# flock-lab/flock

Hardware: AMD Instinct MI355X
Metric: NEXMark rows/sec per node (q3 join, q5 agg) (higher is better)
Workload: dtype int32; 1 GPU; NEXMark q5 hopping(10,5) over 1087 s x 1000000 events/s per GPU; query=q5, input_rows_per_gpu=1000040000, windows_per_gpu=216, parallelism=one GPU, one process

## Files before the change

flock_amd/csrc/q5.hip:

```cpp
#include <algorithm>

#include "sort.hpp"

using namespace flockgpu;

namespace {

constexpr int kQ5Iters = 8;
constexpr int kQ5Tile = kBlock * 4 * kQ5Iters;
constexpr int kHist = 4096;
constexpr int kHistPad = 64;
constexpr int kSlots = kHist / 2;
constexpr int kSlotBits = 11;
static_assert(kSlots == (1 << kSlotBits), "slot bits");
constexpr int kLdsMaxProbe = 24;
constexpr uint32_t kFib = 0x9E3779B1u;
constexpr int kHotMin = 16;
constexpr int kMaxWinPanes = 8;
constexpr uint32_t kWideTile = 0x40000000u;

using u16x2 = unsigned short __attribute__((ext_vector_type(2)));
__device__ __forceinline__ u16x2 as_u16x2(uint32_t w) { return __builtin_bit_cast(u16x2, w); }
__device__ __forceinline__ u16x2 nonzero_u16x2(u16x2 c) {
    uint32_t r;
// ... 835 lines not shown
            const u16x2 one = {1, 1};
            u16x2 pk_a = {0, 0}, pk_b = {0, 0};
            uint32_t sum32 = 0;
            const uint32_t i_first = blockIdx.x * kBlock + threadIdx.x, i_step = gridDim.x * kBlock;
            for (uint32_t i = i_first; i < ng; i += i_step) {
                const int64_t k0 = pd.base + (int64_t)i * G;
                const uint64_t idx = (uint64_t)(k0 - next.base);
                const bool cov = act_b && idx < (uint64_t)next.range;
                const uint4 m4 = *reinterpret_cast<const uint4 *>(mine + (uint64_t)i * 4);
                uint4 o4 = *reinterpret_cast<const uint4 *>(theirs + (cov ? idx / 2 : uint64_t(0)));
                o4.x = cov ? o4.x : 0u;
                o4.y = cov ? o4.y : 0u;
                o4.z = cov ? o4.z : 0u;
                o4.w = cov ? o4.w : 0u;
                const uint32_t mw[4] = {m4.x, m4.y, m4.z, m4.w}, ow[4] = {o4.x, o4.y, o4.z, o4.w};
#pragma unroll
                for (int j = 0; j < 4; ++j) sum32 = __builtin_amdgcn_udot2(as_u16x2(mw[j]), one, sum32, false);
                if (act_b) {
#pragma unroll
                    for (int j = 0; j < 4; ++j) {
                        const u16x2 c = __builtin_elementwise_add_sat(as_u16x2(mw[j]), as_u16x2(ow[j]));
                        pk_b = __builtin_elementwise_max(pk_b, c);
                        groups_b = __builtin_amdgcn_udot2(nonzero_u16x2(c), one, groups_b, false);
                    }
                }
                if (act_a && !((uint64_t)(k0 - prev.base) < (uint64_t)prev.range)) {
#pragma unroll
                    for (int j = 0; j < 4; ++j) {
                        const u16x2 c = as_u16x2(mw[j]);
                        pk_a = __builtin_elementwise_max(pk_a, c);
                        groups_a = __builtin_amdgcn_udot2(nonzero_u16x2(c), one, groups_a, false);
                    }
                }
            }
            sum = sum32;
            best_a = max((uint32_t)pk_a.x, (uint32_t)pk_a.y);
            best_b = max((uint32_t)pk_b.x, (uint32_t)pk_b.y);
            if (best_b == 0xFFFFu) {
                for (uint32_t i = i_first; i < ng; i += i_step) {
                    const uint64_t idx = (uint64_t)(pd.base + (int64_t)i * G - next.base);
                    if (!(idx < (uint64_t)next.range)) continue;
                    uint32_t me[G], o[G];
                    unpack(*reinterpret_cast<const uint4 *>(mine + (uint64_t)i * 4), me);
                    unpack(*reinterpret_cast<const uint4 *>(theirs + idx / 2), o);
#pragma unroll
                    for (int j = 0; j < G; ++j) best_b = max(best_b, me[j] + o[j]);
                }
            }
        }
    }
    if (!packed_done)
    for (uint32_t i = blockIdx.x * kBlock + threadIdx.x; i < ng; i += gridDim.x * kBlock) {
        const int64_t k0 = pd.base + (int64_t)i * G;
        uint32_t me[G];
        unpack(*reinterpret_cast<const uint4 *>(mine + (uint64_t)i * 4), me);
        if (k16 && !SELECT) {
#pragma unroll
            for (int j = 0; j < G; ++j) sum += me[j];
        }
        if (act_b) {
            uint32_t c[G];
#pragma unroll
            for (int j = 0; j < G; ++j) c[j] = me[j];
            const uint64_t idx = (uint64_t)(k0 - next.base);
            if (idx < (uint64_t)next.range) {
                uint32_t o[G];
                unpack(*reinterpret_cast<const uint4 *>(theirs + (k16 ? idx / 2 : idx)), o);
#pragma unroll
                for (int j = 0; j < G; ++j) c[j] += o[j];
            }
            if (tab_b) {
#pragma unroll
                for (int j = 0; j < G; ++j) c[j] += table_find(tb, cap, (uint32_t)(int32_t)(k0 + j));
            }
#pragma unroll
            for (int j = 0; j < G; ++j) take(c[j], (int32_t)(k0 + j), wb, mx_b, best_b, groups_b);
        }
        if (act_a && !((uint64_t)(k0 - prev.base) < (uint64_t)prev.range)) {
            uint32_t c[G];
#pragma unroll
            for (int j = 0; j < G; ++j) c[j] = me[j];
            if (tab_a) {
#pragma unroll
                for (int j = 0; j < G; ++j) c[j] += table_find(ta, cap, (uint32_t)(int32_t)(k0 + j));
            }
#pragma unroll
            for (int j = 0; j < G; ++j) take(c[j], (int32_t)(k0 + j), wa, mx_a, best_a, groups_a);
        }
    }
    if (tab_b && act_b) {
        for (uint32_t sl = blockIdx.x * kBlock + threadIdx.x; sl < cap; sl += gridDim.x * kBlock) {
            const uint64_t e = tb[sl];
            if (!e) continue;
            const int64_t key = (int32_t)(uint32_t)(e >> 32);
            if ((uint64_t)(key - pd.base) < (uint64_t)pd.range || (uint64_t)(key - next.base) < (uint64_t)next.range) continue;
            if (SELECT) {
                if ((uint32_t)e == mx_b) {
                    const uint32_t pos = atomicAdd(cursor, 1u);
                    if (pos < out_cap) {
                        out_win[pos] = wb;
                        out_key[pos] = (int32_t)key;
                    }
                }
            } else {
                best_b = max(best_b, (uint32_t)e);
                groups_b += 1;
            }
        }
    }
    if (!SELECT) {
        const uint32_t ba = wave_max_u32(best_a), bb = wave_max_u32(best_b);
        const uint64_t ga = wave_sum_u64(groups_a), gb = wave_sum_u64(groups_b), gs = k16 ? wave_sum_u64(sum) : 0;
        if (lane_id() == 0) {
            s_best[0][threadIdx.x >> 6] = ba;
            s_best[1][threadIdx.x >> 6] = bb;
            s_groups[0][threadIdx.x >> 6] = ga;
            s_groups[1][threadIdx.x >> 6] = gb;
            s_groups[2][threadIdx.x >> 6] = gs;
        }
        __syncthreads();
        if (threadIdx.x < 2) {
            const int r = threadIdx.x;
            const int32_t w = r == 0 ? wa : wb;
            uint32_t b = 0;
            uint64_t g = 0;
#pragma unroll
            for (int v = 0; v < kWavesPerBlock; ++v) {
                b = max(b, s_best[r][v]);
                g += s_groups[r][v];
            }
            if (w >= 0) {
                if (b) block_max[((size_t)w * 2 + (r == 0 ? 1 : 0)) * gridDim.x + blockIdx.x] = b;
                if (b) atomicMax(reinterpret_cast<unsigned long long *>(&win_max[w]), (unsigned long long)b);
                if (g) atomicAdd(reinterpret_cast<unsigned long long *>(&win_groups[w]), (unsigned long long)g);
            }
        }
        if (k16 && threadIdx.x == 2) {
            uint64_t t = 0;
#pragma unroll
            for (int v = 0; v < kWavesPerBlock; ++v) t += s_groups[2][v];
            if (t) atomicAdd(&pane_sum[p], (unsigned long long)t);
        }
    }
}

constexpr int kFinishThreads = 1024;
constexpr uint32_t kFinishMax = 1024;
__global__ __launch_bounds__(kFinishThreads) void q5_finish_kernel(const uint64_t *__restrict__ meta, uint32_t n_meta, int32_t n_win, const uint64_t *__restrict__ info,
                                                                   const int32_t *__restrict__ slow_list, const int32_t *__restrict__ sel_win,
                                                                   const int32_t *__restrict__ sel_key, uint32_t out_cap, int32_t *__restrict__ out_auction,
                                                                   uint64_t *__restrict__ out_num, uint64_t *__restrict__ h_fin,
                                                                   const unsigned long long *__restrict__ pane_sum, const unsigned long long *__restrict__ tab_rows,
                                                                   const int64_t *__restrict__ seg_off, const int32_t *__restrict__ pane_win_ptr, int32_t n_panes) {
    __shared__ uint64_t s_k[kFinishMax];
    __shared__ uint32_t s_bad;
    const uint32_t *tail = reinterpret_cast<const uint32_t *>(meta + 2 * (size_t)n_win);
    const uint32_t n_sel = tail[0], err = tail[1];
    if (threadIdx.x == 0) s_bad = 0;
    __syncthreads();
    if (pane_sum && (!info || info[2]))
        for (int32_t p = threadIdx.x; p < n_panes; p += kFinishThreads)
            if (pane_win_ptr[p + 1] != pane_win_ptr[p] && pane_sum[p] + tab_rows[p] != (unsigned long long)(seg_off[2 * p + 1] - seg_off[2 * p])) s_bad = 1;
    __syncthreads();
    const uint32_t bad16 = s_bad;
    for (uint32_t i = threadIdx.x; i < n_meta; i += kFinishThreads) h_fin[i] = meta[i];
    if (threadIdx.x < 3) h_fin[n_meta + threadIdx.x] = info ? info[threadIdx.x] : 0;
    if (threadIdx.x == 3) h_fin[n_meta + 3] = (uint64_t)(uint32_t)slow_list[0] | ((uint64_t)bad16 << 32);
    const bool sortable = !err && !bad16 && n_sel <= kFinishMax && n_sel <= out_cap && (!info || info[2]);
    if (threadIdx.x == 4) h_fin[n_meta + 4] = sortable ? 1 : 0;
    int64_t *h_off = reinterpret_cast<int64_t *>(h_fin + n_meta + 5);
    if (!sortable) return;
    uint32_t p2 = 1;
    while (p2 < n_sel) p2 <<= 1;
    if (threadIdx.x < p2)
        s_k[threadIdx.x] = threadIdx.x < n_sel ? ((uint64_t)(uint32_t)sel_win[threadIdx.x] << 32) | ((uint32_t)sel_key[threadIdx.x] ^ 0x80000000u) : ~0ull;
    __syncthreads();
    for (uint32_t k = 2; k <= p2; k <<= 1)
        for (uint32_t j = k >> 1; j > 0; j >>= 1) {
            const uint32_t i = threadIdx.x, l = i ^ j;
            if (i < p2 && l > i) {
                const uint64_t a = s_k[i], b = s_k[l];
                const bool up = (i & k) == 0;
                if ((a > b) == up) {
                    s_k[i] = b;
                    s_k[l] = a;
                }
            }
            __syncthreads();
        }
    if (threadIdx.x < n_sel) {
        const uint64_t e = s_k[threadIdx.x];
        out_auction[threadIdx.x] = (int32_t)((uint32_t)e ^ 0x80000000u);
        out_num[threadIdx.x] = meta[(uint32_t)(e >> 32)];
    }
    for (int32_t w = threadIdx.x; w <= n_win; w += kFinishThreads) {
        uint32_t lo = 0, hi = n_sel;
        while (lo < hi) {
            const uint32_t mid = (lo + hi) >> 1;
            if ((int32_t)(s_k[mid] >> 32) < w) lo = mid + 1;
            else hi = mid;
        }
        h_off[w] = (int64_t)lo;
    }
}

constexpr int kPartItems = 16;
constexpr int kPartTile = kBlock * kPartItems;
constexpr int kPartShift = 13;
constexpr int kPartMaxDigits = 256;

__device__ __forceinline__ uint32_t part_digit(int32_t key, const PaneDesc &pd, uint32_t straggler) {
    const uint64_t idx = (uint64_t)((int64_t)key - pd.base);
    return idx < (uint64_t)pd.range ? (uint32_t)(idx >> kPartShift) : straggler;
}

__global__ __launch_bounds__(kBlock) void q5_part_tile_kernel(const int32_t *__restrict__ auction, SegTiles st, const PaneDesc *__restrict__ panes,
                                                              const int32_t *__restrict__ pane_win_ptr, uint32_t nd, int32_t *__restrict__ off_mat,
                                                              int32_t *__restrict__ keys_out, uint16_t *__restrict__ low_out,
                                                              uint32_t *__restrict__ sample) {
    __shared__ uint32_t s_cnt[kPartMaxDigits];
    __shared__ __attribute__((aligned(16))) uint16_t s_low[kPartTile];
    __shared__ uint32_t s_wave_total[kWavesPerBlock];
    __shared__ int32_t s_red[2 * kWavesPerBlock];
    const int lane = lane_id(), wave = threadIdx.x >> 6;
    s_cnt[threadIdx.x] = 0;
    const int32_t tile = (int32_t)blockIdx.x;
    const TileRange tr = locate_tile(st, tile, kPartTile);
    if (pane_win_ptr[tr.seg] == pane_win_ptr[tr.seg + 1]) return;
    const int32_t t0 = st.tile_first[tr.seg], tiles_p = st.tile_first[tr.seg + 1] - t0;
    int32_t *off = off_mat + (size_t)t0 * (nd + 1) + (tile - t0);
    const PaneDesc pd = panes[tr.seg];
    int32_t k[kPartItems];
#pragma unroll
    for (int it = 0; it < kPartItems / 4; ++it) {
        const int64_t r0 = tr.tile_begin + (int64_t)(it * kBlock + threadIdx.x) * 4;
        if (r0 >= tr.lo && r0 + 4 <= tr.hi) {
            const int4 t = stream_load4(auction + r0);
            k[it * 4 + 0] = t.x; k[it * 4 + 1] = t.y; k[it * 4 + 2] = t.z; k[it * 4 + 3] = t.w;
        } else {
#pragma unroll
            for (int j = 0; j < 4; ++j) k[it * 4 + j] = (r0 + j >= tr.lo && r0 + j < tr.hi) ? auction[r0 + j] : 0;
        }
    }
    __syncthreads();
    uint16_t rank[kPartItems];
    int32_t mn = 0x7fffffff, mx = (int32_t)0x80000000;
#pragma unroll
    for (int i = 0; i < kPartItems; ++i) {
        const int64_t r = tr.tile_begin + (int64_t)((i >> 2) * kBlock + threadIdx.x) * 4 + (i & 3);
        rank[i] = 0;
        if (r >= tr.lo && r < tr.hi) {
            rank[i] = (uint16_t)atomicAdd(&s_cnt[part_digit(k[i], pd, nd - 1)], 1u);
            mn = min(mn, k[i]);
            mx = max(mx, k[i]);
        }
    }
    __syncthreads();
    {
        const uint32_t c = s_cnt[threadIdx.x];
        const uint32_t in = wave_incl_scan_u32(c);
        if (lane == 63) s_wave_total[wave] = in;
        __syncthreads();
        uint32_t o = in - c;
#pragma unroll
        for (int w = 0; w < kWavesPerBlock; ++w) o += w < wave ? s_wave_total[w] : 0u;
        s_cnt[threadIdx.x] = o;
        if (threadIdx.x < nd) off[(size_t)threadIdx.x * tiles_p] = (int32_t)o;
        if (threadIdx.x == 0) off[(size_t)nd * tiles_p] = (int32_t)(tr.hi - tr.lo);
    }
    __syncthreads();
#pragma unroll
    for (int i = 0; i < kPartItems; ++i) {
        const int64_t r = tr.tile_begin + (int64_t)((i >> 2) * kBlock + threadIdx.x) * 4 + (i & 3);
        if (r >= tr.lo && r < tr.hi) {
            const uint32_t d = part_digit(k[i], pd, nd - 1), pos = s_cnt[d] + rank[i];
            if (d == nd - 1) keys_out[(size_t)tile * kPartTile + pos] = k[i];
            else s_low[pos] = (uint16_t)(((uint32_t)k[i] - (uint32_t)pd.base) & ((1u << kPartShift) - 1));
        }
    }
    __syncthreads();
    {
        const uint4 *src = reinterpret_cast<const uint4 *>(s_low);
        uint4 *dst = reinterpret_cast<uint4 *>(low_out + (size_t)tile * kPartTile);
        const uint32_t n16 = ((uint32_t)(tr.hi - tr.lo) + 7u) >> 3;
        for (uint32_t i = threadIdx.x; i < n16; i += kBlock) stream_store4(dst + i, src[i]);
    }
    if ((blockIdx.x & 63u) == 0) {
#pragma unroll
        for (int o = 32; o > 0; o >>= 1) {
            mn = min(mn, __shfl_xor(mn, o, 64));
            mx = max(mx, __shfl_xor(mx, o, 64));
        }
        if (lane == 0) {
            s_red[wave] = mn;
            s_red[kWavesPerBlock + wave] = mx;
        }
        __syncthreads();
        if (threadIdx.x == 0) {
            for (int w = 1; w < kWavesPerBlock; ++w) {
                mn = min(mn, s_red[w]);
                mx = max(mx, s_red[kWavesPerBlock + w]);
            }
            atomicAdd(&sample[0], 1u);
            if (mx >= mn && (uint32_t)mx - (uint32_t)mn < (uint32_t)kHist / 2) atomicAdd(&sample[1], 1u);
        }
    }
}

__global__ __launch_bounds__(kBlock) void q5_bucket_count_kernel(const int32_t *__restrict__ keys, const uint16_t *__restrict__ low, SegTiles st,
                                                                 const PaneDesc *__restrict__ panes,
                                                                 const int32_t *__restrict__ pane_win_ptr, const int32_t *__restrict__ pane_win_idx,
                                                                 uint32_t nd, const int32_t *__restrict__ off_mat, uint32_t *counters, uint64_t *tables,
                                                                 uint32_t cap, uint32_t *tab_used, uint32_t *err) {
    __shared__ uint32_t s_hist[1 << kPartShift];
    const uint32_t d = blockIdx.x;
    const int32_t p = blockIdx.y;
    const int32_t t0 = st.tile_first[p], tiles_p = st.tile_first[p + 1] - t0;
    if (tiles_p == 0 || pane_win_ptr[p] == pane_win_ptr[p + 1]) return;
    const int32_t *lo_row = off_mat + (size_t)t0 * (nd + 1) + (size_t)d * tiles_p, *hi_row = lo_row + tiles_p;
    const PaneDesc pd = panes[p];
    const int lane = lane_id(), wave = threadIdx.x >> 6;
    if (d == nd - 1) {
        FlushArgs f;
        f.wp0 = pane_win_ptr[p];
        f.wp1 = pane_win_ptr[p + 1];
        f.pane = pd;
        f.pane_win_idx = pane_win_idx;
        f.counters = counters;
        f.tables = tables;
        f.cap = cap;
        f.tab_used = tab_used;
        f.err = err;
        for (int32_t t = wave; t < tiles_p; t += kWavesPerBlock) {
            const int32_t a = lo_row[t], b = hi_row[t];
            for (int32_t i = a + lane; i < b; i += 64) emit_pair(keys[(size_t)(t0 + t) * kPartTile + i], 1u, f);
        }
        return;
    }
    {
        uint4 *z = reinterpret_cast<uint4 *>(s_hist);
        for (int i = threadIdx.x; i < (1 << kPartShift) / 4; i += kBlock) z[i] = make_uint4(0, 0, 0, 0);
    }
    __syncthreads();
    auto add = [&](uint32_t bin, bool valid) {
        const uint32_t hot = __builtin_amdgcn_readfirstlane(bin);
        const uint64_t b = __ballot(valid && bin == hot);
        if (valid && bin == hot) {
            if (mbcnt(b) == 0) atomicAdd(&s_hist[hot], (uint32_t)__popcll((unsigned long long)b));
        } else if (valid) {
            atomicAdd(&s_hist[bin], 1u);
        }
    };
// ... 180 lines not shown
        now.insert(now.end(), idx.begin(), idx.end());
        if (sig != now) {
            std::copy(ptr.begin(), ptr.end(), h_ptr);
            std::copy(idx.begin(), idx.end(), h_idx);
            std::copy(role_a.begin(), role_a.end(), h_roles);
            std::copy(role_b.begin(), role_b.end(), h_roles + role_a.size());
            FG_HIP(ctx, hipMemcpyAsync(d_ptr, h_ptr, ptr.size() * sizeof(int32_t), hipMemcpyHostToDevice, ctx->stream));
            if (!idx.empty())
                FG_HIP(ctx, hipMemcpyAsync(d_idx, h_idx, idx.size() * sizeof(int32_t), hipMemcpyHostToDevice, ctx->stream));
            FG_HIP(ctx, hipMemcpyAsync(d_roles, h_roles, 2 * role_a.size() * sizeof(int32_t), hipMemcpyHostToDevice, ctx->stream));
            sig = now;
        }
    }

    int32_t *d_rng = nullptr, *h_rng = nullptr;
    const size_t n_rng = (size_t)2 * kRangeBlocks * std::max(n_panes, 1);
    FG_TRY(arena_get_t(ctx, "q5.pane_range", n_rng + 2, &d_rng));
    FG_TRY(pinned_get_t(ctx, "q5.pane_range", n_rng + 2, &h_rng));
    std::vector<PaneDesc> panes((size_t)std::max(n_panes, 1));
    std::vector<WinDesc> wins((size_t)std::max(n_win, 1));
    for (auto &p : panes) p = PaneDesc{0, 0, 0, 0};
    for (int w = 0; w < n_win; ++w) wins[w] = WinDesc{0, 0, win->win_pane_lo[w], win->win_pane_hi[w], 0};
    uint64_t cnt_total = 0, scan_total = 0;
    bool dense = st.n_tiles > 0 && n_win > 0 && max_win_panes <= kMaxWinPanes;
    std::vector<int64_t> &hint = ctx->host_i64[weight ? "q5.layout_hint.weighted" : "q5.layout_hint"];
    if (hint.size() != 3) hint.assign(3, 0);
    const uint64_t budget = std::max<uint64_t>(uint64_t(256) << 20, (uint64_t)covered_rows * 4 * 2);
    if (dense) {
        LaunchScope ls(ctx, "q5_range_kernel");
        hipLaunchKernelGGL(q5_range_kernel, dim3(kRangeBlocks, (unsigned)n_panes), dim3(kBlock), 0, ctx->stream, auction, rows, st.seg_off, d_rng);
    }
    FG_TRY(check_launch(ctx, "q5_range_kernel"));
    std::vector<int64_t> &wide_hint = ctx->host_i64["q5.wide_hint"];
    if (wide_hint.size() != 1) wide_hint.assign(1, 0);
    bool wide_mode = wide_hint[0] != 0 && !weight && !part && dense;
    bool wide_ran = false;
    bool speculate = dense && !part && hint[2] && hint[0] > 0 && !wide_mode;
    auto host_layout = [&]() -> int {
        FG_HIP(ctx, hipMemcpyAsync(h_rng, d_rng, sizeof(int32_t) * n_rng, hipMemcpyDeviceToHost, ctx->stream));
        FG_HIP(ctx, hipStreamSynchronize(ctx->stream));
        cnt_total = scan_total = 0;
        for (int p = 0; p < n_panes && dense; ++p) {
            if (ptr[p + 1] == ptr[p] || se[p] <= sb[p]) continue;
            int64_t lo = INT64_MAX, hi = INT64_MIN;
            for (int b = 0; b < kRangeBlocks; ++b) {
                lo = std::min<int64_t>(lo, h_rng[((size_t)p * kRangeBlocks + b) * 2]);
                hi = std::max<int64_t>(hi, h_rng[((size_t)p * kRangeBlocks + b) * 2 + 1]);
            }
            if (lo > hi) continue;
            int64_t base = 0, range = 0;
            if (!q5_pane_layout(lo, hi, &base, &range)) { dense = false; break; }
            panes[p] = PaneDesc{base, cnt_total, (uint32_t)range, 0};
            cnt_total += (uint64_t)range;
        }
        for (int w = 0; w < n_win && dense; ++w) {
            int64_t lo = INT64_MAX, hi = INT64_MIN;
            for (int p = win->win_pane_lo[w]; p < win->win_pane_hi[w]; ++p)
                if (panes[p].range) {
                    lo = std::min(lo, panes[p].base);
                    hi = std::max(hi, panes[p].base + (int64_t)panes[p].range);
                }
            if (lo >= hi) continue;
            if (hi - lo >= (int64_t(1) << 31)) { dense = false; break; }
            wins[w].base = lo;
            wins[w].range = (uint32_t)(hi - lo);
            scan_total += (uint64_t)(hi - lo);
        }
        if (dense && (cnt_total * 4 > budget || scan_total * 4 > 2 * budget)) dense = false;
        return FLOCKGPU_OK;
    };
    if (dense && !speculate) FG_TRY(host_layout());
    PaneDesc *d_panes = nullptr, *h_panes = nullptr;
    WinDesc *d_wins = nullptr, *h_wins = nullptr;
    FG_TRY(arena_get_t(ctx, "q5.panes", panes.size(), &d_panes));
    FG_TRY(pinned_get_t(ctx, "q5.panes", panes.size(), &h_panes));
    FG_TRY(arena_get_t(ctx, "q5.wins", wins.size(), &d_wins));
    FG_TRY(pinned_get_t(ctx, "q5.wins", wins.size(), &h_wins));
    uint64_t *d_info = nullptr, *h_info = nullptr;
    FG_TRY(arena_get_t(ctx, "q5.layout_info", 4, &d_info));
    FG_TRY(pinned_get_t(ctx, "q5.layout_info", 4, &h_info));
    auto upload_layout = [&]() -> int {
        if (!dense) {
            cnt_total = scan_total = 0;
            for (auto &p : panes) p = PaneDesc{0, 0, 0, 0};
            for (int w = 0; w < n_win; ++w) wins[w] = WinDesc{0, 0, win->win_pane_lo[w], win->win_pane_hi[w], 0};
        }
        std::copy(panes.begin(), panes.end(), h_panes);
        std::copy(wins.begin(), wins.end(), h_wins);
        ctx->host_i64["q5.wins_sig"].clear();
        FG_HIP(ctx, hipMemcpyAsync(d_panes, h_panes, panes.size() * sizeof(PaneDesc), hipMemcpyHostToDevice, ctx->stream));
        FG_HIP(ctx, hipMemcpyAsync(d_wins, h_wins, wins.size() * sizeof(WinDesc), hipMemcpyHostToDevice, ctx->stream));
        return FLOCKGPU_OK;
    };
    uint32_t *counters = nullptr;
    uint64_t capacity = 0;
    std::vector<int64_t> &preclean = ctx->host_i64["q5.preclean"];
    if (preclean.size() != 2) preclean.assign(2, 0);
    LayoutArgs lay{};
    uint64_t clean_upto = 0;
    const bool c16 = !weight && !part && !wide_mode && hop2 && ctx->host_i64["q5.no_c16"].empty();
    auto words_of = [&](uint64_t n_counters) -> uint64_t { return c16 ? (n_counters + 1) / 2 : n_counters; };
    if (speculate) {
        FG_TRY(arena_get_t(ctx, "q5.counters", (size_t)words_of((uint64_t)hint[0] + (uint64_t)hint[0] / 8) + 8, &counters));
        capacity = (ctx->arena["q5.counters"].cap / sizeof(uint32_t) - 8) * (c16 ? 2 : 1);
        if (preclean[0] == (int64_t)reinterpret_cast<uintptr_t>(counters)) clean_upto = (uint64_t)preclean[1];
        {
            std::vector<int64_t> &wsig = ctx->host_i64["q5.wins_sig"];
            std::vector<int64_t> wnow;
            wnow.reserve((size_t)2 * n_win + 2);
            wnow.push_back((int64_t)reinterpret_cast<uintptr_t>(d_wins));
            for (int w = 0; w < n_win; ++w) {
                wnow.push_back(win->win_pane_lo[w]);
                wnow.push_back(win->win_pane_hi[w]);
            }
            if (wsig != wnow) {
                std::copy(wins.begin(), wins.end(), h_wins);
                FG_HIP(ctx, hipMemcpyAsync(d_wins, h_wins, wins.size() * sizeof(WinDesc), hipMemcpyHostToDevice, ctx->stream));
                wsig = wnow;
            }
        }
        lay = LayoutArgs{d_rng, d_ptr, st.seg_off, n_panes, n_win, capacity, budget, d_panes, d_wins, d_info};
        cnt_total = (uint64_t)hint[0];
        scan_total = (uint64_t)hint[1];
    } else {
        FG_TRY(upload_layout());
        FG_TRY(arena_get_t(ctx, "q5.counters", (size_t)words_of(cnt_total) + 8, &counters));
    }
    preclean[0] = preclean[1] = 0;

    const size_t n_meta = (size_t)2 * n_win + 1 + ((size_t)n_win + 1) / 2 + 1;
    const size_t n_meta_all = n_meta + (size_t)2 * std::max(n_panes, 0);
    uint64_t *d_meta = nullptr, *h_meta = nullptr;
    FG_TRY(arena_get_t(ctx, "q5.meta", n_meta_all, &d_meta));
    unsigned long long *d_pane_sum = reinterpret_cast<unsigned long long *>(d_meta + n_meta), *d_tab_rows = d_pane_sum + std::max(n_panes, 0);
    FG_TRY(pinned_get_t(ctx, "q5.meta", n_meta, &h_meta));
    uint32_t *d_cursor = reinterpret_cast<uint32_t *>(d_meta + 2 * n_win), *d_err = d_cursor + 1, *d_used = d_cursor + 2;

    unsigned long long *d_wsum = nullptr, *h_wsum = nullptr;
    if (weight && n_panes > 0) {
        FG_TRY(arena_get_t(ctx, "q5.pane_weight", (size_t)n_panes + 1, &d_wsum));
        FG_TRY(pinned_get_t(ctx, "q5.pane_weight", (size_t)n_panes + 1, &h_wsum));
    }
    double rpg = ctx->q5_rows_per_group < 1.0 ? 1.0 : ctx->q5_rows_per_group;
    uint64_t cap64 = dense ? 1024 : std::max<uint64_t>(1024, (uint64_t)((double)max_win_rows / rpg * 2.0) + 64);
    uint32_t out_cap = 1u << 16;
    std::vector<int32_t> h_win, h_key;
    uint32_t n_sel = 0;
    const int32_t *sel_win = nullptr, *sel_key = nullptr;
    bool fin_sorted = false;
    const int64_t *fin_off = nullptr;
    const int32_t *fin_auction = nullptr;
    const uint64_t *fin_num = nullptr;
    uint32_t h_slow_count = 0;
    for (int attempt = 0;; ++attempt) {
        if (attempt > 8 || cap64 >= (uint64_t(1) << 31))
            return fail(ctx, FLOCKGPU_ERR_CAPACITY, "q5: hash table capacity %llu still overflows", (unsigned long long)cap64);
        const uint32_t cap = (uint32_t)cap64;
        const uint64_t *spec_info = speculate ? d_info : nullptr;
        uint64_t *tables = nullptr;
        FG_TRY(arena_get_t(ctx, "q5.tables", (size_t)cap * std::max(n_win, 1), &tables));
        int32_t *o_win = nullptr, *o_key = nullptr, *slow_list = nullptr;
        FG_TRY(arena_get_t(ctx, "q5.sel_win", out_cap, &o_win));
        FG_TRY(arena_get_t(ctx, "q5.sel_key", out_cap, &o_key));
        FG_TRY(arena_get_t(ctx, "q5.slow_list", (size_t)st.n_tiles + 2, &slow_list));
        const uint64_t per_win = n_win > 0 ? std::max<uint64_t>(cap, scan_total / n_win / 4) : cap;
        const bool pane_walk = hop2;
        const uint64_t per_pane = n_panes > 0 ? std::max<uint64_t>(cap, cnt_total / (uint64_t)n_panes / 4) : cap;
        const int hop2_blocks = c16 ? 16 : 32;
        const unsigned gx = (unsigned)std::min<int64_t>(std::max<int64_t>(div_up((int64_t)(pane_walk ? per_pane : per_win), kBlock * 2), 1), pane_walk ? hop2_blocks : 64);
        uint32_t *block_max = nullptr;
        const uint64_t n_block_max = (uint64_t)gx * std::max(n_win, 1) * (pane_walk ? 2 : 1);
        FG_TRY(arena_get_t(ctx, "q5.block_max", (size_t)n_block_max, &block_max));
        {
            const uint64_t clear_words = std::max<uint64_t>({words_of(speculate ? capacity : cnt_total), (uint64_t)cap * n_win, (uint64_t)n_meta_all, n_block_max});
            const unsigned cg = (unsigned)std::max<int64_t>(1, std::min<int64_t>(div_up((int64_t)clear_words / 4 + 1, kBlock), (int64_t)ctx->num_cus * 16));
            {
                LaunchScope ls(ctx, "q5_clear_kernel");
                hipLaunchKernelGGL(q5_clear_kernel, dim3(cg), dim3(kBlock), 0, ctx->stream, counters, speculate ? capacity : cnt_total,
                                   (attempt == 0 && speculate) ? (clean_upto & ~uint64_t(3)) : uint64_t(0), tables, (uint64_t)cap * n_win, d_meta, (uint64_t)n_meta_all,
                                   slow_list, block_max, n_block_max, c16 ? 1 : 0, speculate ? lay : LayoutArgs{}, (const uint64_t *)nullptr);
                if (speculate) clean_upto = std::max(clean_upto, words_of(capacity));
            }
            FG_TRY(check_launch(ctx, "q5_clear_kernel"));
        }
        if (d_wsum) FG_HIP(ctx, hipMemsetAsync(d_wsum, 0, sizeof(unsigned long long) * (size_t)n_panes, ctx->stream));
        uint32_t nd = 0;
        if (wide_mode && dense) {
            uint32_t max_range = 0;
            for (int p = 0; p < n_panes; ++p) max_range = std::max(max_range, panes[(size_t)p].range);
            nd = (uint32_t)div_up((int64_t)max_range, int64_t(1) << kPartShift) + 1;
        }
        const bool wide = wide_mode && dense && nd >= 2 && nd <= (uint32_t)kPartMaxDigits && st.n_tiles > 0 && n_win > 0;
        wide_ran = wide;
        uint32_t *d_sample = nullptr, *h_sample = nullptr;
        FG_TRY(arena_get_t(ctx, "q5.part_sample", 4, &d_sample));
        FG_TRY(pinned_get_t(ctx, "q5.part_sample", 4, &h_sample));
        h_sample[0] = h_sample[1] = 0;
        if (wide) {
            SegTiles st4;
            FG_TRY(build_seg_tiles(ctx, "q5.part", sb.data(), se.data(), n_panes, kPartTile, &st4));
            const int64_t slots = (int64_t)st4.n_tiles * (nd + 1);
            if (slots >= (int64_t(1) << 31)) return fail(ctx, FLOCKGPU_ERR_UNSUPPORTED, "q5: too many (pane, digit, tile) slots for the partition pass");
            int32_t *off_mat = nullptr, *part_keys = nullptr;
            uint16_t *part_low = nullptr;
            FG_TRY(arena_get_t(ctx, "q5.part_hist", (size_t)slots + 4, &off_mat));
            FG_TRY(arena_get_t(ctx, "q5.part_keys", (size_t)st4.n_tiles * kPartTile + 4, &part_keys));
            FG_TRY(arena_get_t(ctx, "q5.part_low", (size_t)st4.n_tiles * kPartTile + 8, &part_low));
            FG_HIP(ctx, hipMemsetAsync(d_sample, 0, 2 * sizeof(uint32_t), ctx->stream));
            {
                LaunchScope ls(ctx, "q5_part_tile_kernel");
                hipLaunchKernelGGL(q5_part_tile_kernel, dim3((unsigned)st4.n_tiles), dim3(kBlock), 0, ctx->stream, auction, st4, d_panes, d_ptr, nd, off_mat, part_keys,
                                   part_low, d_sample);
            }
            FG_TRY(check_launch(ctx, "q5_part_tile_kernel"));
            {
                LaunchScope ls(ctx, "q5_bucket_count_kernel");
                hipLaunchKernelGGL(q5_bucket_count_kernel, dim3(nd, (unsigned)n_panes), dim3(kBlock), 0, ctx->stream, part_keys, part_low, st4, d_panes, d_ptr, d_idx, nd,
                                   off_mat, counters, tables, cap, d_used, d_err);
            }
            FG_TRY(check_launch(ctx, "q5_bucket_count_kernel"));
            FG_HIP(ctx, hipMemcpyAsync(h_sample, d_sample, 2 * sizeof(uint32_t), hipMemcpyDeviceToHost, ctx->stream));
        } else if (st.n_tiles > 0 && n_win > 0) {
            {
                LaunchScope ls(ctx, "q5_count_kernel");
                hipLaunchKernelGGL(weight ? q5_count_kernel<true> : q5_count_kernel<false>, dim3((unsigned)st.n_tiles), dim3(kBlock), 0,
                                   ctx->stream, auction, weight, st, d_panes, d_ptr, d_idx, counters, tables, cap, d_used, d_err,
                                   slow_list, spec_info, d_wsum, c16 ? 1 : 0, c16 ? d_tab_rows : (unsigned long long *)nullptr);
            }
            FG_TRY(check_launch(ctx, "q5_count_kernel"));
            if (d_wsum) FG_HIP(ctx, hipMemcpyAsync(h_wsum, d_wsum, sizeof(unsigned long long) * (size_t)n_panes, hipMemcpyDeviceToHost, ctx->stream));
            {
                LaunchScope ls(ctx, "q5_count_slow_kernel");
                const unsigned gs = (unsigned)std::min<int64_t>(st.n_tiles, (int64_t)ctx->num_cus * 8);
                hipLaunchKernelGGL(weight ? q5_count_slow_kernel<true> : q5_count_slow_kernel<false>, dim3(gs), dim3(kBlock), 0,
                                   ctx->stream, auction, weight, st, d_panes, d_ptr, d_idx, counters, tables, cap, d_used, d_err,
                                   slow_list, spec_info, c16 ? 1 : 0, c16 ? d_tab_rows : (unsigned long long *)nullptr);
            }
            FG_TRY(check_launch(ctx, "q5_count_slow_kernel"));
        }
        if (part) {
            const int64_t tab0 = ((int64_t)cnt_total + 3) & ~int64_t(3);
            std::vector<int64_t> xb((size_t)2 * n_win), xe((size_t)2 * n_win);
            for (int w = 0; w < n_win; ++w) {
                xb[2 * w] = (int64_t)panes[w].cnt_off;
                xe[2 * w] = (int64_t)panes[w].cnt_off + (int64_t)panes[w].range;
                xb[2 * w + 1] = tab0 + (int64_t)w * cap;
                xe[2 * w + 1] = xb[2 * w + 1] + cap;
            }
            SegTiles sx;
            FG_TRY(build_seg_tiles(ctx, "q5.partial", xb.data(), xe.data(), 2 * n_win, kFlagTile, &sx));
            uint32_t *x_flags = nullptr, *x_counts = nullptr;
            uint64_t *x_base = nullptr;
            int64_t *d_xoff = nullptr, *h_xoff = nullptr;
            FG_TRY(arena_get_t(ctx, "q5.partial_flags", (size_t)sx.n_tiles * kBlock + 4, &x_flags));
            FG_TRY(arena_get_t(ctx, "q5.partial_counts", (size_t)sx.n_tiles * kWavesPerBlock + 4, &x_counts));
            FG_TRY(arena_get_t(ctx, "q5.partial_base", (size_t)sx.n_tiles + 1, &x_base));
            FG_TRY(arena_get_t(ctx, "q5.partial_off", (size_t)2 * n_win + 1, &d_xoff));
            FG_TRY(pinned_get_t(ctx, "q5.partial_off", (size_t)2 * n_win + 1, &h_xoff));
            if (sx.n_tiles > 0) {
                LaunchScope ls(ctx, "q5_partial_flag_kernel");
                hipLaunchKernelGGL(q5_partial_flag_kernel, dim3((unsigned)sx.n_tiles), dim3(kBlock), 0, ctx->stream, sx, counters, tables,
                                   tab0, x_flags, x_counts);
            }
            FG_TRY(check_launch(ctx, "q5_partial_flag_kernel"));
            FG_TRY(launch_tile_scan(ctx, x_counts, sx.n_tiles, x_base, sx.tile_first, sx.n_seg, d_xoff));
            FG_HIP(ctx, hipMemcpyAsync(h_xoff, d_xoff, sizeof(int64_t) * ((size_t)2 * n_win + 1), hipMemcpyDeviceToHost, ctx->stream));
            FG_HIP(ctx, hipMemcpyAsync(h_meta, d_meta, sizeof(uint64_t) * n_meta, hipMemcpyDeviceToHost, ctx->stream));
            FG_HIP(ctx, hipStreamSynchronize(ctx->stream));
            if (reinterpret_cast<const uint32_t *>(h_meta + 2 * n_win)[1]) {
                cap64 *= 4;
                continue;
            }
            const int64_t n_out = h_xoff[2 * n_win];
            if (n_out >= (int64_t(1) << 31)) return fail(ctx, FLOCKGPU_ERR_UNSUPPORTED, "q5 partial: more than 2^31 groups");
            int32_t *p_key = nullptr;
            uint32_t *p_cnt = nullptr;
            FG_TRY(arena_get_t(ctx, "q5.partial_key", (size_t)n_out + 4, &p_key));
            FG_TRY(arena_get_t(ctx, "q5.partial_cnt", (size_t)n_out + 4, &p_cnt));
            if (sx.n_tiles > 0 && n_out > 0) {
                LaunchScope ls(ctx, "q5_partial_emit_kernel");
                hipLaunchKernelGGL(q5_partial_emit_kernel, dim3((unsigned)sx.n_tiles), dim3(kBlock), 0, ctx->stream, sx, x_flags, x_counts,
                                   x_base, counters, tables, tab0, d_panes, p_key, p_cnt);
            }
            FG_TRY(check_launch(ctx, "q5_partial_emit_kernel"));
            std::vector<int64_t> &poffs = ctx->host_i64["q5.partial_pane_offsets"];
            poffs.resize((size_t)n_win + 1);
            for (int w = 0; w <= n_win; ++w) poffs[w] = h_xoff[2 * w];
            part->auction = p_key;
            part->count = p_cnt;
            part->pane_out_offsets = poffs.data();
            part->rows = n_out;
            return FLOCKGPU_OK;
        }
        if (n_win > 0 && pane_walk) {
            {
                LaunchScope ls(ctx, "q5_max_kernel");
                hipLaunchKernelGGL((c16 ? q5_hop2_scan_kernel<false, true> : q5_hop2_scan_kernel<false, false>), dim3(gx, (unsigned)n_panes), dim3(kBlock), 0, ctx->stream, d_panes, d_roles,
                                   d_roles + role_a.size(), counters, tables, cap, d_used, d_meta, d_meta + n_win, block_max, d_cursor, out_cap, o_win, o_key, spec_info, d_pane_sum);
            }
            FG_TRY(check_launch(ctx, "q5_max_kernel"));
            {
                LaunchScope ls(ctx, "q5_select_kernel");
                hipLaunchKernelGGL((c16 ? q5_hop2_scan_kernel<true, true> : q5_hop2_scan_kernel<true, false>), dim3(gx, (unsigned)n_panes), dim3(kBlock), 0, ctx->stream, d_panes, d_roles,
                                   d_roles + role_a.size(), counters, tables, cap, d_used, d_meta, d_meta + n_win, block_max, d_cursor, out_cap, o_win, o_key, spec_info, d_pane_sum);
            }
            FG_TRY(check_launch(ctx, "q5_select_kernel"));
        } else if (n_win > 0) {
            {
                LaunchScope ls(ctx, "q5_max_kernel");
                hipLaunchKernelGGL(q5_scan_kernel<false>, dim3(gx, (unsigned)n_win), dim3(kBlock), 0, ctx->stream, d_wins,
                                   d_panes, counters, tables, cap, d_used, d_meta, d_meta + n_win, block_max, d_cursor, out_cap,
                                   o_win, o_key, spec_info);
            }
            FG_TRY(check_launch(ctx, "q5_max_kernel"));
            {
                LaunchScope ls(ctx, "q5_select_kernel");
                hipLaunchKernelGGL(q5_scan_kernel<true>, dim3(gx, (unsigned)n_win), dim3(kBlock), 0, ctx->stream, d_wins,
                                   d_panes, counters, tables, cap, d_used, d_meta, d_meta + n_win, block_max, d_cursor, out_cap,
                                   o_win, o_key, spec_info);
            }
            FG_TRY(check_launch(ctx, "q5_select_kernel"));
        }
        constexpr uint32_t kSpecWinners = 4096;
        uint64_t *h_fin = nullptr;
        int32_t *fin_a = nullptr;
        uint64_t *fin_n = nullptr;
        FG_TRY(pinned_get_t(ctx, "q5.finish", n_meta + 8 + (size_t)n_win + 2, &h_fin));
        FG_TRY(arena_get_t(ctx, "q5.out_auction", (size_t)kFinishMax + 1, &fin_a));
        FG_TRY(arena_get_t(ctx, "q5.out_num", (size_t)kFinishMax + 1, &fin_n));
        const bool poll = !d_wsum && !wide;
        if (poll) pinned_pending(h_fin, (int)(n_meta + 5 + (size_t)n_win + 1));
        {
            LaunchScope ls(ctx, "q5_finish_kernel");
            hipLaunchKernelGGL(q5_finish_kernel, dim3(1), dim3(kFinishThreads), 0, ctx->stream, d_meta, (uint32_t)n_meta, n_win, spec_info, slow_list, o_win, o_key, out_cap,
                               fin_a, fin_n, h_fin, c16 && pane_walk ? d_pane_sum : (const unsigned long long *)nullptr, d_tab_rows, st.seg_off, d_ptr, n_panes);
        }
        FG_TRY(check_launch(ctx, "q5_finish_kernel"));
        if (speculate && dense) {
            LaunchScope ls(ctx, "q5_clear_kernel");
            const unsigned cg = (unsigned)std::max<int64_t>(1, std::min<int64_t>(div_up((int64_t)words_of(cnt_total) / 4 + 1, kBlock), (int64_t)ctx->num_cus * 16));
            hipLaunchKernelGGL(q5_clear_kernel, dim3(cg), dim3(kBlock), 0, ctx->stream, counters, capacity, uint64_t(0), (uint64_t *)nullptr,
                               uint64_t(0), (uint64_t *)nullptr, uint64_t(0), slow_list, (uint32_t *)nullptr, uint64_t(0), c16 ? 1 : 0, LayoutArgs{}, d_info);
        }
        FG_TRY(check_launch(ctx, "q5_clear_kernel"));
        if (poll) {
            FG_TRY(wait_pinned(ctx, h_fin, (int)(n_meta + 5)));
            if (h_fin[n_meta + 4]) FG_TRY(wait_pinned(ctx, h_fin + n_meta + 5, n_win + 1));
        } else
            FG_HIP(ctx, hipStreamSynchronize(ctx->stream));
        std::copy(h_fin, h_fin + n_meta, h_meta);
        if (speculate) std::copy(h_fin + n_meta, h_fin + n_meta + 3, h_info);
        h_slow_count = (uint32_t)h_fin[n_meta + 3];
        if (h_fin[n_meta + 3] >> 32) {
            ctx->host_i64["q5.no_c16"].assign(1, 1);
            return q5_run(ctx, auction, weight, rows, win, out, part);
        }
        fin_sorted = h_fin[n_meta + 4] != 0;
        fin_off = reinterpret_cast<const int64_t *>(h_fin + n_meta + 5);
        if (speculate) {
            if (!h_info[2]) {
                speculate = false;
                hint[2] = 0;
                FG_TRY(host_layout());
                FG_TRY(upload_layout());
                FG_TRY(arena_get_t(ctx, "q5.counters", (size_t)words_of(cnt_total) + 8, &counters));
                cap64 = dense ? 1024 : std::max<uint64_t>(1024, (uint64_t)((double)max_win_rows / rpg * 2.0) + 64);
                --attempt;
                continue;
            }
            cnt_total = h_info[0];
            scan_total = h_info[1];
        }
        if (h_wsum) {
            for (int w = 0; w < n_win; ++w) {
                unsigned long long tot = 0;
                for (int p = win->win_pane_lo[w]; p < win->win_pane_hi[w]; ++p) tot += h_wsum[p];
                if (tot >= (1ull << 32))
                    return fail(ctx, FLOCKGPU_ERR_UNSUPPORTED, "q5 weighted: the counts of window %d add up to %llu >= 2^32 (32-bit counters)", w, tot);
            }
        }
        const uint32_t *tail = reinterpret_cast<const uint32_t *>(h_meta + 2 * n_win);
        n_sel = tail[0];
        if (tail[1]) {
            cap64 *= 4;
            continue;
        }
        if (n_sel > out_cap) {
            out_cap = n_sel + 1024;
            continue;
        }
        h_win.resize(n_sel);
        h_key.resize(n_sel);
        if (fin_sorted) {
            fin_auction = fin_a;
            fin_num = fin_n;
        } else if (n_sel <= kSpecWinners) {
            FG_HIP(ctx, hipMemcpyAsync(h_win.data(), o_win, sizeof(int32_t) * n_sel, hipMemcpyDeviceToHost, ctx->stream));
            FG_HIP(ctx, hipMemcpyAsync(h_key.data(), o_key, sizeof(int32_t) * n_sel, hipMemcpyDeviceToHost, ctx->stream));
            FG_HIP(ctx, hipStreamSynchronize(ctx->stream));
        } else {
            sel_win = o_win;
            sel_key = o_key;
        }
        break;
    }
    hint[0] = (int64_t)cnt_total;
    hint[1] = (int64_t)scan_total;
    hint[2] = dense ? 1 : 0;
    if (!weight && !part) {
        uint32_t *h_sample = nullptr;
        FG_TRY(pinned_get_t(ctx, "q5.part_sample", 4, &h_sample));
        if (wide_mode && !wide_ran) wide_hint[0] = 0;
        else if (wide_mode && h_sample[0]) wide_hint[0] = (uint64_t)h_sample[1] * 4 >= (uint64_t)h_sample[0] * 3 ? 0 : 1;
        else if (!wide_mode && dense && st.n_tiles > 64) wide_hint[0] = (int64_t)h_slow_count * 4 > (int64_t)st.n_tiles ? 1 : 0;
    }
    {
        double best = 1e30;
        for (int w = 0; w < n_win; ++w) {
            const int64_t rows = win->pane_row_offsets[win->win_pane_hi[w]] - win->pane_row_offsets[win->win_pane_lo[w]];
            const uint64_t g = h_meta[n_win + w];
            if (g) best = std::min(best, (double)rows / (double)g);
        }
        if (best < 1e30) ctx->q5_rows_per_group = best;
    }
    std::vector<int64_t> &offs = ctx->host_i64["q5.win_out_offsets"];
    std::vector<uint64_t> &wmax = ctx->host_u64["q5.win_max"], &wgrp = ctx->host_u64["q5.win_groups"];
    offs.assign((size_t)n_win + 1, 0);
    wmax.assign(h_meta, h_meta + n_win);
    wgrp.assign(h_meta + n_win, h_meta + 2 * n_win);
    if (fin_sorted) {
        offs.assign(fin_off, fin_off + n_win + 1);
        out->auction = fin_auction;
        out->num = fin_num;
        out->win_out_offsets = offs.data();
        out->win_max = wmax.data();
        out->win_groups = wgrp.data();
        out->rows = n_sel;
    } else
    if (sel_key) {
        int32_t *d_mm = nullptr, *h_mm = nullptr, *k1 = nullptr, *w_in = nullptr, *w2 = nullptr, *d_oa = nullptr;
        uint32_t *v1 = nullptr, *v2 = nullptr;
        uint64_t *d_on = nullptr;
        int64_t *d_off = nullptr, *h_off = nullptr;
        FG_TRY(arena_get_t(ctx, "q5.ord_minmax", 4, &d_mm));
        FG_TRY(pinned_get_t(ctx, "q5.ord_minmax", 4, &h_mm));
        FG_TRY(key_min_max(ctx, sel_key, n_sel, d_mm));
        FG_HIP(ctx, hipMemcpyAsync(h_mm, d_mm, 2 * sizeof(int32_t), hipMemcpyDeviceToHost, ctx->stream));
        FG_HIP(ctx, hipStreamSynchronize(ctx->stream));
        int bits = 1, wbits = 1;
        while (bits < 32 && (((uint64_t)((int64_t)h_mm[1] - (int64_t)h_mm[0])) >> bits)) ++bits;
        while (wbits < 31 && ((uint32_t)n_win >> wbits)) ++wbits;
        FG_TRY(radix_sort_pairs(ctx, "q5.ord_key", sel_key, nullptr, n_sel, h_mm[0], bits, &k1, &v1));
        FG_TRY(arena_get_t(ctx, "q5.ord_win_in", (size_t)n_sel + 4, &w_in));
        FG_TRY(gather_i32(ctx, sel_win, reinterpret_cast<const int32_t *>(v1), n_sel, w_in));
        FG_TRY(radix_sort_pairs(ctx, "q5.ord_win", w_in, v1, n_sel, 0, wbits, &w2, &v2));
        FG_TRY(arena_get_t(ctx, "q5.out_auction", (size_t)n_sel + 1, &d_oa));
        FG_TRY(arena_get_t(ctx, "q5.out_num", (size_t)n_sel + 1, &d_on));
        FG_TRY(arena_get_t(ctx, "q5.ord_off", (size_t)n_win + 2, &d_off));
        FG_TRY(pinned_get_t(ctx, "q5.ord_off", (size_t)n_win + 2, &h_off));
        FG_TRY(gather_i32(ctx, sel_key, reinterpret_cast<const int32_t *>(v2), n_sel, d_oa));
        hipLaunchKernelGGL(q5_winner_num_kernel, dim3((unsigned)div_up((int64_t)n_sel, kBlock)), dim3(kBlock), 0, ctx->stream, w2,
                           d_meta, (int64_t)n_sel, d_on);
        FG_TRY(check_launch(ctx, "q5_winner_num_kernel"));
        FG_TRY(sorted_key_offsets(ctx, w2, n_sel, n_win, d_off));
        FG_HIP(ctx, hipMemcpyAsync(h_off, d_off, sizeof(int64_t) * ((size_t)n_win + 1), hipMemcpyDeviceToHost, ctx->stream));
        FG_HIP(ctx, hipStreamSynchronize(ctx->stream));
        offs.assign(h_off, h_off + n_win + 1);
        out->auction = d_oa;
        out->num = d_on;
        out->win_out_offsets = offs.data();
        out->win_max = wmax.data();
        out->win_groups = wgrp.data();
        out->rows = n_sel;
        return FLOCKGPU_OK;
    }
    if (!fin_sorted) {
    std::vector<uint32_t> order(n_sel);
    for (uint32_t i = 0; i < n_sel; ++i) order[i] = i;
    std::sort(order.begin(), order.end(), [&](uint32_t a, uint32_t b) {
        return h_win[a] != h_win[b] ? h_win[a] < h_win[b] : h_key[a] < h_key[b];
    });
    int32_t *h_oa = nullptr;
    uint64_t *h_on = nullptr;
    FG_TRY(pinned_get_t(ctx, "q5.out_auction", (size_t)n_sel + 1, &h_oa));
    FG_TRY(pinned_get_t(ctx, "q5.out_num", (size_t)n_sel + 1, &h_on));
    for (uint32_t i = 0; i < n_sel; ++i) {
        const uint32_t s = order[i];
        h_oa[i] = h_key[s];
        h_on[i] = wmax[h_win[s]];
        offs[h_win[s] + 1] += 1;
    }
    for (int w = 0; w < n_win; ++w) offs[w + 1] += offs[w];
    int32_t *d_oa = nullptr;
    uint64_t *d_on = nullptr;
    FG_TRY(arena_get_t(ctx, "q5.out_auction", (size_t)n_sel + 1, &d_oa));
    FG_TRY(arena_get_t(ctx, "q5.out_num", (size_t)n_sel + 1, &d_on));
    if (n_sel) {
        FG_HIP(ctx, hipMemcpyAsync(d_oa, h_oa, sizeof(int32_t) * n_sel, hipMemcpyHostToDevice, ctx->stream));
        FG_HIP(ctx, hipMemcpyAsync(d_on, h_on, sizeof(uint64_t) * n_sel, hipMemcpyHostToDevice, ctx->stream));
    }
    out->auction = d_oa;
    out->num = d_on;
    out->win_out_offsets = offs.data();
    out->win_max = wmax.data();
    out->win_groups = wgrp.data();
    out->rows = n_sel;
    }
    if (speculate && dense && cnt_total > 0) {
        preclean[0] = (int64_t)reinterpret_cast<uintptr_t>(counters);
        preclean[1] = (int64_t)std::max<uint64_t>(clean_upto, words_of(cnt_total));
    }
    return FLOCKGPU_OK;
}

namespace flockgpu {

int q5_partial_by_tile(flockgpu_ctx *ctx, const flockgpu_bid_cols *bid, const flockgpu_windows *win, Q5TilePartial *out) {
    *out = Q5TilePartial{};
    FG_TRY(check_windows(ctx, win, bid->rows, "q5 partial"));
    if (bid->rows > 0 && !bid->auction) return fail(ctx, FLOCKGPU_ERR_INVALID, "q5 partial: null auction column");
    if (reinterpret_cast<uintptr_t>(bid->auction) & 15) return fail(ctx, FLOCKGPU_ERR_UNSUPPORTED, "q5: auction column must be 16-byte aligned");
    if (bid->rows >= (int64_t(1) << 31)) return fail(ctx, FLOCKGPU_ERR_UNSUPPORTED, "q5 partial: more than 2^31 rows per call");
    FG_HIP(ctx, hipSetDevice(ctx->device));
    const int n_panes = win->n_panes;
    std::vector<char> used((size_t)std::max(n_panes, 1), 0);
    for (int w = 0; w < win->n_windows; ++w)
        for (int p = win->win_pane_lo[w]; p < win->win_pane_hi[w]; ++p) used[(size_t)p] = 1;
    std::vector<int64_t> sb((size_t)n_panes), se((size_t)n_panes);
    for (int p = 0; p < n_panes; ++p) {
        sb[(size_t)p] = win->pane_row_offsets[p];
        se[(size_t)p] = win->pane_row_offsets[p + 1];
    }
    SegTiles st;
    FG_TRY(build_seg_tiles(ctx, "q5.tile_panes", sb.data(), se.data(), n_panes, kQ5Tile, &st));
    int64_t *d_reg = nullptr, *h_reg = nullptr;
    uint32_t *d_cur = nullptr, *h_cur = nullptr;
    int32_t *o_key = nullptr;
    uint32_t *o_cnt = nullptr;
    FG_TRY(arena_get_t(ctx, "q5.tile_region", (size_t)n_panes + 1, &d_reg));
    FG_TRY(pinned_get_t(ctx, "q5.tile_region", (size_t)n_panes + 1, &h_reg));
    FG_TRY(arena_get_t(ctx, "q5.tile_cursor", (size_t)n_panes + 1, &d_cur));
    FG_TRY(pinned_get_t(ctx, "q5.tile_cursor", (size_t)n_panes + 1, &h_cur));
    FG_TRY(arena_get_t(ctx, "q5.tile_key", (size_t)bid->rows + 4, &o_key));
    FG_TRY(arena_get_t(ctx, "q5.tile_cnt", (size_t)bid->rows + 4, &o_cnt));
    for (int p = 0; p < n_panes; ++p) h_reg[p] = used[(size_t)p] ? sb[(size_t)p] : -1;
    FG_HIP(ctx, hipMemcpyAsync(d_reg, h_reg, sizeof(int64_t) * (size_t)std::max(n_panes, 1), hipMemcpyHostToDevice, ctx->stream));
    FG_HIP(ctx, hipMemsetAsync(d_cur, 0, sizeof(uint32_t) * ((size_t)n_panes + 1), ctx->stream));
    int64_t max_tiles = 0;
    for (int p = 0; p < n_panes; ++p)
        if (se[(size_t)p] > sb[(size_t)p]) max_tiles = std::max(max_tiles, div_up(se[(size_t)p] - (sb[(size_t)p] & ~int64_t(3)), (int64_t)kQ5Tile));
    if (max_tiles * n_panes >= (int64_t(1) << 31)) return fail(ctx, FLOCKGPU_ERR_UNSUPPORTED, "q5 partial: too many (pane, tile) pairs");
    if (st.n_tiles > 0) {
        LaunchScope ls(ctx, "q5_partial_tile_kernel");
        hipLaunchKernelGGL(q5_partial_tile_kernel, dim3((unsigned)(max_tiles * n_panes)), dim3(kBlock), 0, ctx->stream, bid->auction, st, d_reg, d_cur, o_key,
                           o_cnt);
    }
    FG_TRY(check_launch(ctx, "q5_partial_tile_kernel"));
    FG_HIP(ctx, hipMemcpyAsync(h_cur, d_cur, sizeof(uint32_t) * (size_t)std::max(n_panes, 1), hipMemcpyDeviceToHost, ctx->stream));
    FG_HIP(ctx, hipStreamSynchronize(ctx->stream));
    out->auction = o_key;
    out->count = o_cnt;
// ... 47 lines not shown
```

Before: 1308 billion rows/s.

## Skip slow-tile count kernel speculatively and replace bitonic sort with rank sort

Adds a host-side streak counter that skips launching q5_count_slow_kernel in speculative mode once several consecutive calls had no slow tiles. If a skipped run then reports slow tiles, it reruns the attempt and doubles the backoff window. Separately, the finish kernel's bitonic sort with many barriers is replaced by a one-pass rank-by-counting sort into a second shared buffer. The skip risks a costly retry whenever slow tiles reappear, and the rank sort does O(n^2) comparisons per block.

```diff
diff --git a/flock_amd/csrc/q5.hip b/flock_amd/csrc/q5.hip
--- a/flock_amd/csrc/q5.hip
+++ b/flock_amd/csrc/q5.hip
@@ -1011,7 +1011,7 @@
                                                                    uint64_t *__restrict__ out_num, uint64_t *__restrict__ h_fin,
                                                                    const unsigned long long *__restrict__ pane_sum, const unsigned long long *__restrict__ tab_rows,
                                                                    const int64_t *__restrict__ seg_off, const int32_t *__restrict__ pane_win_ptr, int32_t n_panes) {
-    __shared__ uint64_t s_k[kFinishMax];
+    __shared__ uint64_t s_k[kFinishMax], s_sorted[kFinishMax];
     __shared__ uint32_t s_bad;
     const uint32_t *tail = reinterpret_cast<const uint32_t *>(meta + 2 * (size_t)n_win);
     const uint32_t n_sel = tail[0], err = tail[1];
@@ -1029,34 +1029,29 @@
     if (threadIdx.x == 4) h_fin[n_meta + 4] = sortable ? 1 : 0;
     int64_t *h_off = reinterpret_cast<int64_t *>(h_fin + n_meta + 5);
     if (!sortable) return;
-    uint32_t p2 = 1;
-    while (p2 < n_sel) p2 <<= 1;
-    if (threadIdx.x < p2)
-        s_k[threadIdx.x] = threadIdx.x < n_sel ? ((uint64_t)(uint32_t)sel_win[threadIdx.x] << 32) | ((uint32_t)sel_key[threadIdx.x] ^ 0x80000000u) : ~0ull;
+    const uint32_t n_pad = (n_sel + 3u) & ~3u;
+    uint64_t own = ~0ull;
+    if (threadIdx.x < n_pad) {
+        if (threadIdx.x < n_sel) own = ((uint64_t)(uint32_t)sel_win[threadIdx.x] << 32) | ((uint32_t)sel_key[threadIdx.x] ^ 0x80000000u);
+        s_k[threadIdx.x] = own;
+    }
     __syncthreads();
-    for (uint32_t k = 2; k <= p2; k <<= 1)
-        for (uint32_t j = k >> 1; j > 0; j >>= 1) {
-            const uint32_t i = threadIdx.x, l = i ^ j;
-            if (i < p2 && l > i) {
-                const uint64_t a = s_k[i], b = s_k[l];
-                const bool up = (i & k) == 0;
-                if ((a > b) == up) {
-                    s_k[i] = b;
-                    s_k[l] = a;
-                }
-            }
-            __syncthreads();
-        }
     if (threadIdx.x < n_sel) {
-        const uint64_t e = s_k[threadIdx.x];
-        out_auction[threadIdx.x] = (int32_t)((uint32_t)e ^ 0x80000000u);
-        out_num[threadIdx.x] = meta[(uint32_t)(e >> 32)];
-    }
+        uint32_t rank = 0;
+        for (uint32_t j = 0; j < n_pad; j += 4) {
+#pragma unroll
+            for (uint32_t u = 0; u < 4; ++u) rank += s_k[j + u] < own ? 1u : 0u;
+        }
+        s_sorted[rank] = own;
+        out_auction[rank] = (int32_t)((uint32_t)own ^ 0x80000000u);
+        out_num[rank] = meta[(uint32_t)(own >> 32)];
+    }
+    __syncthreads();
     for (int32_t w = threadIdx.x; w <= n_win; w += kFinishThreads) {
         uint32_t lo = 0, hi = n_sel;
         while (lo < hi) {
             const uint32_t mid = (lo + hi) >> 1;
-            if ((int32_t)(s_k[mid] >> 32) < w) lo = mid + 1;
+            if ((int32_t)(s_sorted[mid] >> 32) < w) lo = mid + 1;
             else hi = mid;
         }
         h_off[w] = (int64_t)lo;
@@ -1543,6 +1538,9 @@
     const int32_t *fin_auction = nullptr;
     const uint64_t *fin_num = nullptr;
     uint32_t h_slow_count = 0;
+    std::vector<int64_t> &slow_rec = ctx->host_i64["q5.slow_rec"];
+    if (slow_rec.size() != 2) slow_rec = {0, 1};
+    bool skip_slow = speculate && !weight && !part && !wide_mode && slow_rec[0] >= slow_rec[1];
     for (int attempt = 0;; ++attempt) {
         if (attempt > 8 || cap64 >= (uint64_t(1) << 31))
             return fail(ctx, FLOCKGPU_ERR_CAPACITY, "q5: hash table capacity %llu still overflows", (unsigned long long)cap64);
@@ -1620,7 +1618,7 @@
             }
             FG_TRY(check_launch(ctx, "q5_count_kernel"));
             if (d_wsum) FG_HIP(ctx, hipMemcpyAsync(h_wsum, d_wsum, sizeof(unsigned long long) * (size_t)n_panes, hipMemcpyDeviceToHost, ctx->stream));
-            {
+            if (!(skip_slow && speculate)) {
                 LaunchScope ls(ctx, "q5_count_slow_kernel");
                 const unsigned gs = (unsigned)std::min<int64_t>(st.n_tiles, (int64_t)ctx->num_cus * 8);
                 hipLaunchKernelGGL(weight ? q5_count_slow_kernel<true> : q5_count_slow_kernel<false>, dim3(gs), dim3(kBlock), 0,
@@ -1742,6 +1740,12 @@
         std::copy(h_fin, h_fin + n_meta, h_meta);
         if (speculate) std::copy(h_fin + n_meta, h_fin + n_meta + 3, h_info);
         h_slow_count = (uint32_t)h_fin[n_meta + 3];
+        if (skip_slow && speculate && h_slow_count) {
+            skip_slow = false;
+            slow_rec[0] = 0;
+            slow_rec[1] = std::min<int64_t>(slow_rec[1] * 2, 1024);
+            continue;
+        }
         if (h_fin[n_meta + 3] >> 32) {
             ctx->host_i64["q5.no_c16"].assign(1, 1);
             return q5_run(ctx, auction, weight, rows, win, out, part);
@@ -1798,6 +1802,7 @@
     hint[0] = (int64_t)cnt_total;
     hint[1] = (int64_t)scan_total;
     hint[2] = dense ? 1 : 0;
+    if (!weight && !part) slow_rec[0] = (wide_mode || h_slow_count) ? 0 : slow_rec[0] + 1;
     if (!weight && !part) {
         uint32_t *h_sample = nullptr;
         FG_TRY(pinned_get_t(ctx, "q5.part_sample", 4, &h_sample));
```

Measured after the change: 1319 billion rows/s, median of 6. Within noise of the previous version (+0.8%).
